# 001camellia/Speech-Imagery-EEG

Measured on AMD Instinct MI355X. Metric: epochs/sec (B=256, C=122, T=1000) IGN 3-class, higher is better.
Workload: dtype f32

## Files before the change

### speech-imagery-eeg_amd/csrc/ign_clconv.h

```cpp
#pragma once
#include "ign_common.h"

typedef float f32x16 __attribute__((ext_vector_type(16)));
#define MFMA32(a, b, c) __builtin_amdgcn_mfma_f32_32x32x2f32((a), (b), (c), 0, 0, 0)

__device__ __forceinline__ int acc_row16(int r, int h) { return (r & 3) + 8 * (r >> 2) + 4 * h; }

constexpr int TM = 128, TN = 128, KC = 16;
constexpr int NT_PITCH = KC + 4;
constexpr int TN_PITCH = 128 + 8;

struct RowMap {
    int rows_logical;
    int row0;
    int row_pitch;
    long long sample_pitch;
};
__device__ __forceinline__ long long row_off(const RowMap& rm, int m) {
    const int s = m / rm.rows_logical;
    const int r = m - s * rm.rows_logical;
    return (long long)s * rm.sample_pitch + (long long)(rm.row0 + r) * rm.row_pitch;
}

template <int V> struct VecT;
template <> struct VecT<1> { typedef float T; };
template <> struct VecT<2> { typedef float2 T; };
template <> struct VecT<4> { typedef float4 T; };

template <int V>
__device__ __forceinline__ void vload(float (&d)[V], const float* p) {
    if (V == 4) { const float4 t = *reinterpret_cast<const float4*>(p); d[0] = t.x; d[1] = t.y; d[2] = t.z; d[3] = t.w; }
    else if (V == 2) { const float2 t = *reinterpret_cast<const float2*>(p); d[0] = t.x; d[1] = t.y; }
    else d[0] = *p;
}
template <int V>
__device__ __forceinline__ void vstore(float* p, const float (&d)[V]) {
    if (V == 4) *reinterpret_cast<float4*>(p) = make_float4(d[0], d[1], d[2], d[3]);
    else if (V == 2) *reinterpret_cast<float2*>(p) = make_float2(d[0], d[1]);
    else *p = d[0];
}

enum { EPI_BIAS_STATS = 0, EPI_MASK_STATS = 1, EPI_GELU_BWD = 2 };

__device__ __forceinline__ float ign_gelu_grad(float u) {
    const float cdf = 0.5f * (1.f + erff(u * 0.70710678118654752f));
    const float pdf = 0.3989422804014327f * expf(-0.5f * u * u);
    return fmaf(u, pdf, cdf);
}

struct GemmNTArgs {
    const float* A; RowMap am; int K;
    const float* Bt; int ldb;
    float* C; int M, N;
    const float* bias;
    const float* pro_a; const float* pro_b; int pro_c;
    float* part;
    const float* ey; const float* ea; const float* eb; const float* emean; const float* einv;
    int mtiles, ntiles;
    const unsigned short* B3; int Kp;
    float* amax_out;
};

template <int EPI, bool FULL, bool SC = false>
__device__ __forceinline__ void nt_epilogue_body(const GemmNTArgs& a, const f32x16 (&acc)[2][2], float (&s1)[2], float (&s2)[2],
                                                 int m0, int n0, int m_lim, float osc = 1.f) {
    const int lane = threadIdx.x & 63, wave = threadIdx.x >> 6;
    const int l31 = lane & 31, h = lane >> 5;
    const int wm = wave & 1, wn = wave >> 1;
    float amax = 0.f;
#pragma unroll
    for (int j = 0; j < 2; ++j) {
        const int n = n0 + wn * 64 + j * 32 + l31;
        const bool n_ok = FULL || n < a.N;
        const int nc = n_ok ? n : a.N - 1;
        const float bv = (EPI == EPI_BIAS_STATS && a.bias) ? a.bias[nc] : 0.f;
        float ea = 0.f, eb = 0.f, em = 0.f, ei = 0.f;
        if (EPI == EPI_MASK_STATS) { ea = a.ea[nc]; eb = a.eb[nc]; em = a.emean[nc]; ei = a.einv[nc]; }
#pragma unroll
        for (int i = 0; i < 2; ++i) {
            const int mb = m0 + wm * 64 + i * 32;
            float yv[16];
            if (EPI == EPI_MASK_STATS || EPI == EPI_GELU_BWD) {
#pragma unroll
                for (int r = 0; r < 16; ++r) {
                    const int m = mb + acc_row16(r, h);
                    const int mc = FULL ? m : min(m, m_lim - 1);
                    yv[r] = a.ey[(long long)mc * a.N + nc];
                }
            }
#pragma unroll
            for (int r = 0; r < 16; ++r) {
                const int m = mb + acc_row16(r, h);
                const bool ok = FULL || (n_ok && m < m_lim);
                float v = SC ? acc[i][j][r] * osc : acc[i][j][r];
                if (EPI == EPI_BIAS_STATS) {
                    v += bv;
                    if (ok) { s1[j] += v; s2[j] = fmaf(v, v, s2[j]); }
                } else if (EPI == EPI_GELU_BWD) {
                    v *= ign_gelu_grad(yv[r]);
                } else {
                    v = (fmaf(ea, yv[r], eb) > 0.f) ? v : 0.f;
                    if (ok) { s1[j] += v; s2[j] = fmaf(v, (yv[r] - em) * ei, s2[j]); }
                }
                if (ok) a.C[(long long)m * a.N + n] = v;
                if (SC && ok) amax = fmaxf(amax, fabsf(v));
            }
        }
    }
    if (SC && a.amax_out) {
#pragma unroll
        for (int o = 32; o > 0; o >>= 1) amax = fmaxf(amax, __shfl_xor(amax, o, 64));
        if (lane == 0) ign_atomic_absmax(a.amax_out, amax);
    }
}

template <int EPI, bool SC = false>
__device__ __forceinline__ void nt_epilogue(const GemmNTArgs& a, const f32x16 (&acc)[2][2], float* red, int mt, int m0, int n0,
                                            int m_lim, float osc = 1.f) {
    const int tid = threadIdx.x, lane = tid & 63, wave = tid >> 6;
    const int l31 = lane & 31, h = lane >> 5;
    const int wm = wave & 1, wn = wave >> 1;
    float s1[2] = {0.f, 0.f}, s2[2] = {0.f, 0.f};
    if (m0 + TM <= m_lim && n0 + TN <= a.N) nt_epilogue_body<EPI, true, SC>(a, acc, s1, s2, m0, n0, m_lim, osc);
    else nt_epilogue_body<EPI, false, SC>(a, acc, s1, s2, m0, n0, m_lim, osc);
    if (a.part) {
#pragma unroll
        for (int j = 0; j < 2; ++j) {
            s1[j] += __shfl_xor(s1[j], 32, 64);
            s2[j] += __shfl_xor(s2[j], 32, 64);
            if (h == 0) {
                const int col = wn * 64 + j * 32 + l31;
                red[(wm * 2 + 0) * TN + col] = s1[j];
                red[(wm * 2 + 1) * TN + col] = s2[j];
            }
        }
        __syncthreads();
        if (tid < TN && n0 + tid < a.N) {
            a.part[((long long)mt * 2 + 0) * a.N + n0 + tid] = red[0 * TN + tid] + red[2 * TN + tid];
            a.part[((long long)mt * 2 + 1) * a.N + n0 + tid] = red[1 * TN + tid] + red[3 * TN + tid];
        }
    }
}


struct ConvX6Args {
    GemmNTArgs g;
    long long sample_pitch;
    int rows_in;
    int cin, cp, k;
    int trows;
    int tps;
    int nprod;
    const float* bound_a;
    const float* bound_b;
};

__device__ __forceinline__ float ign_pow2_scale(const float* bound) {
    if (!bound) return 1.f;
    const float b = *bound;
    if (!(b > 0.f) || !(b < INFINITY)) return 1.f;
    int e;
    (void)frexpf(b, &e);
    e = 14 - e;
    e = e < -60 ? -60 : (e > 60 ? 60 : e);
    return ldexpf(1.f, e);
}

inline int ign_vec_width(int c) { return (c % 4 == 0) ? 4 : (c % 2 == 0) ? 2 : 1; }

int ign_clconv_launch_x6t(const ConvX6Args& a, int epi, int V, bool pro, hipStream_t s);
int ign_clconv_launch_wgrad_reduce(const float* part, float* dw_oik, int nsplit, int Co, int Ci, int k, hipStream_t s);
```

### speech-imagery-eeg_amd/csrc/ign_clconv_x6.hip

```cpp
#include "ign_clconv.h"

typedef __bf16 bf16x8 __attribute__((ext_vector_type(8)));
constexpr int X6_PITCH = KC + 8;
constexpr int X6_PLANE = TM * X6_PITCH;
constexpr int X6_BLOCK = 3 * TN * KC;

typedef float f32x2 __attribute__((ext_vector_type(2)));
typedef __bf16 bf16x2 __attribute__((ext_vector_type(2)));
__device__ __forceinline__ void split3_pair(f32x2 v, bf16x2& x0, bf16x2& x1, bf16x2& x2) {
    x0 = __builtin_convertvector(v, bf16x2);
    f32x2 r = v - __builtin_convertvector(x0, f32x2);
    x1 = __builtin_convertvector(r, bf16x2);
    r -= __builtin_convertvector(x1, f32x2);
    x2 = __builtin_convertvector(r, bf16x2);
}
template <int V>
__device__ __forceinline__ void split3_store(const float (&t)[V], __bf16* d, int plane);
template <>
__device__ __forceinline__ void split3_store<1>(const float (&t)[1], __bf16* d, int plane);
__device__ __forceinline__ void split3(float v, __bf16& x0, __bf16& x1, __bf16& x2) {
    x0 = (__bf16)v;
    float r = v - (float)x0;
    x1 = (__bf16)r;
    r -= (float)x1;
    x2 = (__bf16)r;
}
template <>
__device__ __forceinline__ void split3_store<1>(const float (&t)[1], __bf16* d, int plane) {
    __bf16 x0, x1, x2;
    split3(t[0], x0, x1, x2);
    d[0] = x0; d[plane] = x1; d[2 * plane] = x2;
}
template <>
__device__ __forceinline__ void split3_store<2>(const float (&t)[2], __bf16* d, int plane) {
    bf16x2 x0, x1, x2;
    split3_pair(f32x2{t[0], t[1]}, x0, x1, x2);
    *reinterpret_cast<bf16x2*>(d) = x0;
    *reinterpret_cast<bf16x2*>(d + plane) = x1;
    *reinterpret_cast<bf16x2*>(d + 2 * plane) = x2;
}
template <>
__device__ __forceinline__ void split3_store<4>(const float (&t)[4], __bf16* d, int plane) {
    typedef __bf16 bf16x4 __attribute__((ext_vector_type(4)));
    bf16x2 a0, a1, a2, b0, b1, b2;
    split3_pair(f32x2{t[0], t[1]}, a0, a1, a2);
    split3_pair(f32x2{t[2], t[3]}, b0, b1, b2);
    *reinterpret_cast<bf16x4*>(d) = __builtin_shufflevector(a0, b0, 0, 1, 2, 3);
    *reinterpret_cast<bf16x4*>(d + plane) = __builtin_shufflevector(a1, b1, 0, 1, 2, 3);
    *reinterpret_cast<bf16x4*>(d + 2 * plane) = __builtin_shufflevector(a2, b2, 0, 1, 2, 3);
}

typedef _Float16 f16x2 __attribute__((ext_vector_type(2)));
typedef _Float16 f16x4 __attribute__((ext_vector_type(4)));
typedef _Float16 f16x8 __attribute__((ext_vector_type(8)));
__device__ __forceinline__ void split2h_pair(f32x2 v, f16x2& x0, f16x2& x1) {
    x0 = __builtin_convertvector(v, f16x2);
    x1 = __builtin_convertvector(v - __builtin_convertvector(x0, f32x2), f16x2);
}
template <int V>
__device__ __forceinline__ void split2h_store(const float (&t)[V], __bf16* d, int plane) {
    _Float16* dh = reinterpret_cast<_Float16*>(d);
    if constexpr (V == 1) {
        const _Float16 x0 = (_Float16)t[0];
        dh[0] = x0; dh[plane] = (_Float16)(t[0] - (float)x0);
    } else if constexpr (V == 2) {
        f16x2 x0, x1;
        split2h_pair(f32x2{t[0], t[1]}, x0, x1);
        *reinterpret_cast<f16x2*>(dh) = x0;
        *reinterpret_cast<f16x2*>(dh + plane) = x1;
    } else {
        f16x2 a0, a1, b0, b1;
        split2h_pair(f32x2{t[0], t[1]}, a0, a1);
        split2h_pair(f32x2{t[2], t[3]}, b0, b1);
        *reinterpret_cast<f16x4*>(dh) = __builtin_shufflevector(a0, b0, 0, 1, 2, 3);
        *reinterpret_cast<f16x4*>(dh + plane) = __builtin_shufflevector(a1, b1, 0, 1, 2, 3);
    }
}

template <int V, int NP>
__device__ __forceinline__ void split_store(const float (&t)[V], __bf16* d, int plane) {
    if constexpr (NP == 3) {
        split3_store<V>(t, d, plane);
    } else if constexpr (NP == 2) {
        split2h_store<V>(t, d, plane);
    } else if constexpr (V == 1) {
        d[0] = (__bf16)t[0];
    } else if constexpr (V == 2) {
        *reinterpret_cast<bf16x2*>(d) = __builtin_convertvector(f32x2{t[0], t[1]}, bf16x2);
    } else {
        typedef __bf16 bf16x4 __attribute__((ext_vector_type(4)));
        const bf16x2 a = __builtin_convertvector(f32x2{t[0], t[1]}, bf16x2), b = __builtin_convertvector(f32x2{t[2], t[3]}, bf16x2);
        *reinterpret_cast<bf16x4*>(d) = __builtin_shufflevector(a, b, 0, 1, 2, 3);
    }
}

template <int NP>
__device__ __forceinline__ f32x16 mfma16(const bf16x8& a, const bf16x8& b, const f32x16& c) {
    if constexpr (NP == 2)
        return __builtin_amdgcn_mfma_f32_32x32x16_f16(__builtin_bit_cast(f16x8, a), __builtin_bit_cast(f16x8, b), c, 0, 0, 0);
    else
        return __builtin_amdgcn_mfma_f32_32x32x16_bf16(a, b, c, 0, 0, 0);
}

#ifndef IGN_H3_WAVES
#define IGN_H3_WAVES 3
#endif
constexpr int X6T_SPAN = TM + 15;
constexpr int X6T_APLANE = X6T_SPAN * X6_PITCH;

template <int NP> struct X6tLds {
    static constexpr int NPL = (NP == 2) ? 2 : 3;
    static constexpr int ABUF = NPL * X6T_APLANE, BBUF = NPL * X6_PLANE;
    static constexpr size_t BYTES = (size_t)2 * (ABUF + BBUF) * sizeof(unsigned short);
};
template <int NP, int EPI> struct X6tWaves { static constexpr int N = (NP == 2 && EPI == EPI_BIAS_STATS) ? IGN_H3_WAVES : 2; };
template <int V, bool PRO, int EPI, int NP>
__global__ void __launch_bounds__(256, (X6tWaves<NP, EPI>::N)) clconv_x6t_kernel(const ConvX6Args ca) {
    const GemmNTArgs& a = ca.g;
    constexpr int VPR = KC / V;
    constexpr int APASS = (X6T_SPAN * VPR + 255) / 256;
    constexpr int X6T_ABUF = X6tLds<NP>::ABUF, X6T_BBUF = X6tLds<NP>::BBUF;
    extern __shared__ __attribute__((aligned(16))) unsigned short smem16[];
    __bf16* Abuf = reinterpret_cast<__bf16*>(smem16);
    __bf16* Bbuf = Abuf + 2 * X6T_ABUF;

    const int nwg = a.mtiles * a.ntiles;
    int lid = blockIdx.x;
    {
        const int per = nwg / 8;
        if (lid < per * 8) lid = (lid & 7) * per + (lid >> 3);
    }
    const int mt = lid / a.ntiles, nt = lid - mt * a.ntiles;
    const int bi = mt / ca.tps, tt = mt - bi * ca.tps;
    const int t0 = tt * TM, n0 = nt * TN;
    const int tid = threadIdx.x, lane = tid & 63, wave = tid >> 6;
    const int l31 = lane & 31, h = lane >> 5;
    const int wm = wave & 1, wn = wave >> 1;
    const int span = TM + ca.k - 1;
    const int nvec = span * VPR;

    const float* abase = a.A + (long long)bi * ca.sample_pitch;
    const int brw = tid >> 1, bh = tid & 1;
    const unsigned short* bsrc = a.B3 + (size_t)nt * (size_t)(ca.cp / KC) * ca.k * X6_BLOCK + (size_t)brw * KC + 8 * bh;
    constexpr size_t bplane = (size_t)TN * KC;

    f32x16 acc[2][2];
#pragma unroll
    for (int i = 0; i < 2; ++i)
#pragma unroll
        for (int j = 0; j < 2; ++j)
#pragma unroll
            for (int r = 0; r < 16; ++r) acc[i][j][r] = 0.f;

    float ra[APASS][V];
    float pa[V], pb[V];
    bool a_ok = false;
    uint4 rb00, rb01 = {}, rb02 = {}, rb10, rb11 = {}, rb12 = {};
    const int ncc = ca.cp / KC;
    const int nstep = ncc * ca.k;

    const float sa = (NP == 2) ? ign_pow2_scale(ca.bound_a) : 1.f;
    const float osc = (NP == 2) ? 1.f / (sa * ign_pow2_scale(ca.bound_b)) : 1.f;
    auto aload = [&](int cc) {
        const int ch = cc * KC + (tid % VPR) * V;
        a_ok = ch < ca.cin;
        if (PRO && a_ok) {
            vload<V>(pa, a.pro_a + ch); vload<V>(pb, a.pro_b + ch);
            if constexpr (NP == 2) {
#pragma unroll
                for (int v = 0; v < V; ++v) { pa[v] *= sa; pb[v] *= sa; }
            }
        }
#pragma unroll
        for (int p = 0; p < APASS; ++p) {
            const int idx = tid + p * 256;
            const int row = idx / VPR;
            if (a_ok && idx < nvec) vload<V>(ra[p], abase + (long long)min(t0 + row, ca.rows_in - 1) * ca.cin + ch);
            else {
#pragma unroll
                for (int v = 0; v < V; ++v) ra[p][v] = 0.f;
            }
        }
    };
    auto astore = [&](int buf) {
        __bf16* st = Abuf + buf * X6T_ABUF;
#pragma unroll
        for (int p = 0; p < APASS; ++p) {
            const int idx = tid + p * 256;
            if (idx < nvec) {
                const int row = idx / VPR, q = idx - row * VPR;
                float tv[V];
#pragma unroll
                for (int v = 0; v < V; ++v) {
                    tv[v] = ra[p][v];
                    if (PRO && a_ok) tv[v] = fmaxf(fmaf(pa[v], tv[v], pb[v]), 0.f);
                    else if (NP == 2) tv[v] *= sa;
                }
                split_store<V, NP>(tv, st + row * X6_PITCH + q * V, X6T_APLANE);
            }
        }
    };
    auto boff = [&](int st) {
        st = min(st, nstep - 1);
        return (size_t)st * X6_BLOCK;
    };
    auto bstore = [&](int buf, const uint4& r0, const uint4& r1, const uint4& r2) {
        __bf16* st = Bbuf + buf * X6T_BBUF + brw * X6_PITCH + 8 * bh;
        *reinterpret_cast<uint4*>(st) = r0;
        if constexpr (NP >= 2) *reinterpret_cast<uint4*>(st + X6_PLANE) = r1;
        if constexpr (NP == 3) *reinterpret_cast<uint4*>(st + 2 * X6_PLANE) = r2;
    };
#define IGN_BLOAD(r0, r1, r2, st)                                                                       \
    do {                                                                                                \
        const size_t off_ = boff(st);                                                                   \
        r0 = *reinterpret_cast<const uint4*>(bsrc + off_);                                              \
        if constexpr (NP >= 2) r1 = *reinterpret_cast<const uint4*>(bsrc + bplane + off_);              \
        if constexpr (NP == 3) r2 = *reinterpret_cast<const uint4*>(bsrc + 2 * bplane + off_);          \
    } while (0)

    aload(0);
    IGN_BLOAD(rb00, rb01, rb02, 0);
    IGN_BLOAD(rb10, rb11, rb12, 1);
    astore(0);
    bstore(0, rb00, rb01, rb02);
    __syncthreads();

    int cc = 0, j = 0;
    auto body = [&](int step, bool odd) {
        if (odd) IGN_BLOAD(rb10, rb11, rb12, step + 2);
        else IGN_BLOAD(rb00, rb01, rb02, step + 2);
        const bool next_span = cc + 1 < ncc;
        if (j == 0 && next_span) aload(cc + 1);
        const __bf16* As = Abuf + (cc & 1) * X6T_ABUF + (wm * 64 + l31 + j) * X6_PITCH + 8 * h;
        const __bf16* Bs = Bbuf + (step & 1) * X6T_BBUF + (wn * 64 + l31) * X6_PITCH + 8 * h;
        bf16x8 af[2][NP], bf[2][NP];
#pragma unroll
        for (int i = 0; i < 2; ++i)
#pragma unroll
            for (int pl = 0; pl < NP; ++pl) {
                af[i][pl] = *reinterpret_cast<const bf16x8*>(As + pl * X6T_APLANE + i * 32 * X6_PITCH);
                bf[i][pl] = *reinterpret_cast<const bf16x8*>(Bs + pl * X6_PLANE + i * 32 * X6_PITCH);
            }
        __builtin_amdgcn_sched_barrier(0);
#define IGN_X6(pa_, pb_)                                                                                   \
        acc[0][0] = mfma16<NP>(af[0][pa_], bf[0][pb_], acc[0][0]);                                         \
        acc[0][1] = mfma16<NP>(af[0][pa_], bf[1][pb_], acc[0][1]);                                         \
        acc[1][0] = mfma16<NP>(af[1][pa_], bf[0][pb_], acc[1][0]);                                         \
        acc[1][1] = mfma16<NP>(af[1][pa_], bf[1][pb_], acc[1][1]);
        if constexpr (NP == 3) { IGN_X6(2, 0) IGN_X6(0, 2) IGN_X6(1, 1) IGN_X6(1, 0) IGN_X6(0, 1) }
        if constexpr (NP == 2) { IGN_X6(1, 0) IGN_X6(0, 1) }
        IGN_X6(0, 0)
#undef IGN_X6
        __builtin_amdgcn_sched_barrier(0);
        if (odd) bstore((step + 1) & 1, rb00, rb01, rb02);
        else bstore((step + 1) & 1, rb10, rb11, rb12);
        if (j + 1 == ca.k) {
            if (next_span) astore((cc + 1) & 1);
            j = 0; ++cc;
        } else {
            ++j;
        }
        __syncthreads();
    };
    for (int step = 0; step < nstep; step += 2) {
        body(step, false);
        if (step + 1 < nstep) body(step + 1, true);
    }
#undef IGN_BLOAD
    const int m0 = bi * ca.trows + t0;
    nt_epilogue<EPI, NP == 2>(a, acc, reinterpret_cast<float*>(smem16), mt, m0, n0, bi * ca.trows + min(ca.trows, t0 + TM), osc);
}

#ifndef IGN_H3W_WAVES
#define IGN_H3W_WAVES 2
#endif
template <int NP> struct X6wLds {
    static constexpr int NPL = NP == 3 ? 3 : (NP == 2 ? 2 : 1);
    static constexpr int ABUF = NPL * TM * X6_PITCH;
    static constexpr int BBUF = 2 * NPL * X6_PLANE;
    static constexpr size_t BYTES = (size_t)2 * (ABUF + BBUF) * sizeof(unsigned short);
    static constexpr int WAVES = NP == 2 ? IGN_H3W_WAVES : 2;
};

template <int NP, int EPI = EPI_BIAS_STATS>
__global__ void __launch_bounds__(512, X6wLds<NP>::WAVES) clconv_x6w_kernel(const ConvX6Args ca) {
    const GemmNTArgs& a = ca.g;
    extern __shared__ __attribute__((aligned(16))) unsigned short smem16[];
    constexpr int X6W_ABUF = X6wLds<NP>::ABUF, X6W_BBUF = X6wLds<NP>::BBUF, NPL = X6wLds<NP>::NPL;
    __bf16* Abuf = reinterpret_cast<__bf16*>(smem16);
    __bf16* Bbuf = Abuf + 2 * X6W_ABUF;
    constexpr int APLANE = TM * X6_PITCH;

    const int ntw = a.N / 256;
    const int nwg = a.mtiles * ntw;
    int lid = blockIdx.x;
    {
        const int per = nwg / 8;
        if (lid < per * 8) lid = (lid & 7) * per + (lid >> 3);
    }
    const int mt = lid / ntw, nw = lid - mt * ntw;
    const int m0 = mt * TM, n0 = nw * 256;
    const int tid = threadIdx.x, lane = tid & 63, wave = tid >> 6;
    const int l31 = lane & 31, h = lane >> 5;
    const int wm = wave & 1, wn = wave >> 1;
    const int ncc = ca.cp / KC;

    f32x16 acc[2][2];
#pragma unroll
    for (int i = 0; i < 2; ++i)
#pragma unroll
        for (int j = 0; j < 2; ++j)
#pragma unroll
            for (int r = 0; r < 16; ++r) acc[i][j][r] = 0.f;

    const int arow = tid >> 2, ach = (tid & 3) * 4;
    const float* ap = a.A + (long long)min(m0 + arow, a.M - 1) * ca.cin + ach;
    float ra0[4], ra1[4];
    const int bt = tid >> 8, brw = (tid & 255) >> 1, bh = tid & 1;
    const unsigned short* bsrc = a.B3 + (size_t)(2 * nw + bt) * (size_t)ncc * X6_BLOCK + (size_t)brw * KC + 8 * bh;
    constexpr size_t bplane = (size_t)TN * KC;
    uint4 rb00, rb01 = {}, rb02 = {}, rb10, rb11 = {}, rb12 = {};

    const float sa = (NP == 2) ? ign_pow2_scale(ca.bound_a) : 1.f;
    const float osc = (NP == 2) ? 1.f / (sa * ign_pow2_scale(ca.bound_b)) : 1.f;
#define IGN_ALOADW(ra_, cc_)                                                                 \
    do {                                                                                     \
        const int c_ = min((cc_), ncc - 1);                                                  \
        if (c_ * KC + ach < ca.cin) vload<4>(ra_, ap + c_ * KC);           \
        else ra_[0] = ra_[1] = ra_[2] = ra_[3] = 0.f;                                        \
    } while (0)
    auto astore = [&](int buf, const float (&r)[4]) {
        if constexpr (NP == 2) {
            const float rs[4] = {r[0] * sa, r[1] * sa, r[2] * sa, r[3] * sa};
            split_store<4, NP>(rs, Abuf + buf * X6W_ABUF + arow * X6_PITCH + ach, APLANE);
        } else {
            split_store<4, NP>(r, Abuf + buf * X6W_ABUF + arow * X6_PITCH + ach, APLANE);
        }
    };
    auto bstore = [&](int buf, const uint4& r0, const uint4& r1, const uint4& r2) {
        __bf16* st = Bbuf + buf * X6W_BBUF + bt * NPL * X6_PLANE + brw * X6_PITCH + 8 * bh;
        *reinterpret_cast<uint4*>(st) = r0;
        if constexpr (NP >= 2) *reinterpret_cast<uint4*>(st + X6_PLANE) = r1;
        if constexpr (NP == 3) *reinterpret_cast<uint4*>(st + 2 * X6_PLANE) = r2;
    };
#define IGN_BLOADW(r0, r1, r2, st)                                                                      \
    do {                                                                                                \
        const size_t off_ = (size_t)min((st), ncc - 1) * X6_BLOCK;                                      \
        r0 = *reinterpret_cast<const uint4*>(bsrc + off_);                                              \
        if constexpr (NP >= 2) r1 = *reinterpret_cast<const uint4*>(bsrc + bplane + off_);              \
        if constexpr (NP == 3) r2 = *reinterpret_cast<const uint4*>(bsrc + 2 * bplane + off_);          \
    } while (0)

    IGN_ALOADW(ra0, 0);
    IGN_BLOADW(rb00, rb01, rb02, 0);
    IGN_ALOADW(ra1, 1);
    IGN_BLOADW(rb10, rb11, rb12, 1);
    astore(0, ra0);
    bstore(0, rb00, rb01, rb02);
    __syncthreads();

    const bool late = wave >= 4;
    auto mm = [&](int step) {
        const __bf16* As = Abuf + (step & 1) * X6W_ABUF + (wm * 64 + l31) * X6_PITCH + 8 * h;
        const __bf16* Bs = Bbuf + (step & 1) * X6W_BBUF + (wn >> 1) * NPL * X6_PLANE + ((wn & 1) * 64 + l31) * X6_PITCH + 8 * h;
        bf16x8 af[2][NP], bf[2][NP];
#pragma unroll
        for (int i = 0; i < 2; ++i)
#pragma unroll
            for (int pl = 0; pl < NP; ++pl) {
                af[i][pl] = *reinterpret_cast<const bf16x8*>(As + pl * APLANE + i * 32 * X6_PITCH);
                bf[i][pl] = *reinterpret_cast<const bf16x8*>(Bs + pl * X6_PLANE + i * 32 * X6_PITCH);
            }
        __builtin_amdgcn_sched_barrier(0);
#define IGN_X6(pa_, pb_)                                                                                   \
        acc[0][0] = mfma16<NP>(af[0][pa_], bf[0][pb_], acc[0][0]);                                         \
        acc[0][1] = mfma16<NP>(af[0][pa_], bf[1][pb_], acc[0][1]);                                         \
        acc[1][0] = mfma16<NP>(af[1][pa_], bf[0][pb_], acc[1][0]);                                         \
        acc[1][1] = mfma16<NP>(af[1][pa_], bf[1][pb_], acc[1][1]);
        if constexpr (NP == 3) { IGN_X6(2, 0) IGN_X6(0, 2) IGN_X6(1, 1) }
        if constexpr (NP >= 2) { IGN_X6(1, 0) IGN_X6(0, 1) }
        IGN_X6(0, 0)
#undef IGN_X6
        __builtin_amdgcn_sched_barrier(0);
    };
    auto body = [&](int step, bool odd) {
        if (odd) { IGN_BLOADW(rb10, rb11, rb12, step + 2); IGN_ALOADW(ra1, step + 2); }
        else { IGN_BLOADW(rb00, rb01, rb02, step + 2); IGN_ALOADW(ra0, step + 2); }
        const bool next = step + 1 < ncc;
        auto st = [&]() {
            if (odd) { bstore((step + 1) & 1, rb00, rb01, rb02); if (next) astore((step + 1) & 1, ra0); }
            else { bstore((step + 1) & 1, rb10, rb11, rb12); if (next) astore((step + 1) & 1, ra1); }
            __builtin_amdgcn_sched_barrier(0);
        };
        if (late) { st(); mm(step); } else { mm(step); st(); }
        __syncthreads();
    };
    for (int step = 0; step < ncc; step += 2) {
        body(step, false);
        if (step + 1 < ncc) body(step + 1, true);
    }
#undef IGN_BLOADW
#undef IGN_ALOADW
    float s1[2] = {0.f, 0.f}, s2[2] = {0.f, 0.f};
    const int m_lim = a.M;
    if (m0 + TM <= m_lim) nt_epilogue_body<EPI, true, NP == 2>(a, acc, s1, s2, m0, n0, m_lim, osc);
    else nt_epilogue_body<EPI, false, NP == 2>(a, acc, s1, s2, m0, n0, m_lim, osc);
}

__device__ __forceinline__ void pack_weights_x3t_body(const float* __restrict__ w, unsigned short* __restrict__ wt3,
                                                      unsigned short* __restrict__ wd3, int Co, int Ci, int k, int Cip, int Cop,
                                                      long long i, const float* __restrict__ bound = nullptr) {
    const long long nf = (long long)((Co + TN - 1) / TN) * (Cip / KC) * k * (TN * KC);
    const long long nd = wd3 ? (long long)((Ci + TN - 1) / TN) * (Cop / KC) * k * (TN * KC) : 0;
    const bool fwd = i < nf;
    if (!fwd && i >= nf + nd) return;
    const long long e = fwd ? i : i - nf;
    const int q = (int)(e % KC);
    long long t = e / KC;
    const int row = (int)(t % TN);
    t /= TN;
    const int j = (int)(t % k);
    t /= k;
    const int ncc = (fwd ? Cip : Cop) / KC;
    const int cc = (int)(t % ncc);
    const int nt = (int)(t / ncc);
    const int n = nt * TN + row, c = cc * KC + q;
    float v = 0.f;
    if (fwd) { if (n < Co && c < Ci) v = w[((long long)n * Ci + c) * k + j]; }
    else     { if (n < Ci && c < Co) v = w[((long long)c * Ci + n) * k + (k - 1 - j)]; }
    const long long blk = ((long long)(nt * ncc + cc) * k + j) * X6_BLOCK + (long long)row * KC + q;
    if (bound) {
        const float sv = v * ign_pow2_scale(bound);
        const _Float16 h0 = (_Float16)sv;
        _Float16* dh = reinterpret_cast<_Float16*>(fwd ? wt3 : wd3) + blk;
        dh[0] = h0; dh[TN * KC] = (_Float16)(sv - (float)h0);
        return;
    }
    __bf16 x0, x1, x2;
    split3(v, x0, x1, x2);
    __bf16* dst = reinterpret_cast<__bf16*>(fwd ? wt3 : wd3) + blk;
    dst[0] = x0; dst[TN * KC] = x1; dst[2 * TN * KC] = x2;
}

__global__ void __launch_bounds__(256) pack_weights_x3t_kernel(const float* __restrict__ w, unsigned short* __restrict__ wt3,
                                                               unsigned short* __restrict__ wd3, int Co, int Ci, int k, int Cip,
                                                               int Cop) {
    pack_weights_x3t_body(w, wt3, wd3, Co, Ci, k, Cip, Cop, (long long)blockIdx.x * 256 + threadIdx.x);
}

constexpr int PACK_LMAX = 8;
struct PackMultiTable {
    const float* w[PACK_LMAX];
    unsigned short* wt3[PACK_LMAX];
    unsigned short* wd3[PACK_LMAX];
    long long* counter[PACK_LMAX];
    const float* bound[PACK_LMAX];
    int Co[PACK_LMAX], Ci[PACK_LMAX], k[PACK_LMAX];
};
__global__ void __launch_bounds__(256) pack_weights_x3t_multi_kernel(const PackMultiTable t) {
    const int l = blockIdx.y;
    if (blockIdx.x == 0 && threadIdx.x == 0 && t.counter[l]) *t.counter[l] += 1;
    pack_weights_x3t_body(t.w[l], t.wt3[l], t.wd3[l], t.Co[l], t.Ci[l], t.k[l], (t.Ci[l] + 15) / 16 * 16, (t.Co[l] + 15) / 16 * 16,
                          (long long)blockIdx.x * 256 + threadIdx.x, t.bound[l]);
}

typedef short s16x4 __attribute__((ext_vector_type(4)));
typedef short s16x8 __attribute__((ext_vector_type(8)));
constexpr int WG_PITCH = 64 + 32;

struct WgradX6Args {
    const float* dy; long long dy_sample_pitch; int dy_row0;
    const float* x; long long x_sample_pitch;
    const float* pro_a; const float* pro_b;
    float* part;
    int B, Tin, Tout, Ci, Co, k;
    int cps;
    int nunits, nsplit, citiles;
    const float* bound_dy; const float* bound_x;
};

__device__ __forceinline__ bf16x8 lds_tr8(const __bf16* p0, const __bf16* p1) {
    typedef __attribute__((address_space(3))) s16x4* lds_p;
    const s16x4 lo = __builtin_amdgcn_ds_read_tr16_b64_v4i16((lds_p)(p0));
    const s16x4 hi = __builtin_amdgcn_ds_read_tr16_b64_v4i16((lds_p)(p1));
    const s16x8 v = __builtin_shufflevector(lo, hi, 0, 1, 2, 3, 4, 5, 6, 7);
    return __builtin_bit_cast(bf16x8, v);
}

template <int KT, int NR, int VX, bool PRO, int NP>
__global__ void __launch_bounds__(256, ((NP == 2 && KT <= 5) ? IGN_H3_WAVES : 2)) clconv_wgrad_x6_kernel(const WgradX6Args a) {
    constexpr int RU = 16 * NR;
    constexpr int SPAN = RU + KT - 1;
    constexpr int PPLANE = RU * WG_PITCH, QPLANE = SPAN * WG_PITCH;
    constexpr int NPL = (NP == 2) ? 2 : 3;
    constexpr int STAGE = NPL * (PPLANE + QPLANE);
    constexpr int XVPR = 64 / VX;
    constexpr int XPASS = (SPAN * XVPR + 255) / 256;
    constexpr int DPASS = NR;
    extern __shared__ __attribute__((aligned(16))) unsigned short smem16[];
    __bf16* smem = reinterpret_cast<__bf16*>(smem16);

    const int tile = blockIdx.x;
    const int cot = tile / a.citiles, cit = tile - cot * a.citiles;
    const int co0 = cot * 64, ci0 = cit * 64;
    const int split = blockIdx.y;
    const int per = (a.nunits + a.nsplit - 1) / a.nsplit;
    const int u_begin = split * per, u_end = min(a.nunits, u_begin + per);

    const int tid = threadIdx.x, lane = tid & 63, wave = tid >> 6;
    const int l31 = lane & 31, h = lane >> 5;
    const int wco = wave & 1, wci = wave >> 1;

    const int dr = tid >> 4, dc = (tid & 15) * 4;
    const bool d_ok = co0 + dc < a.Co;
    const int xq = (tid % XVPR) * VX;
    const bool x_ok = ci0 + xq < a.Ci;
    float pa[VX], pb[VX];
    if (PRO && x_ok) { vload<VX>(pa, a.pro_a + ci0 + xq); vload<VX>(pb, a.pro_b + ci0 + xq); }
    const float sdy = (NP == 2) ? ign_pow2_scale(a.bound_dy) : 1.f;
    const float sx = (NP == 2) ? ign_pow2_scale(a.bound_x) : 1.f;
    const float osc = (NP == 2) ? 1.f / (sdy * sx) : 1.f;
    if (NP == 2 && PRO && x_ok) {
#pragma unroll
        for (int v = 0; v < VX; ++v) { pa[v] *= sx; pb[v] *= sx; }
    }

    f32x16 acc[KT];
#pragma unroll
    for (int j = 0; j < KT; ++j)
#pragma unroll
        for (int r = 0; r < 16; ++r) acc[j][r] = 0.f;

    float rd[DPASS][4], rx[XPASS][VX];
    auto gload = [&](int u) {
        const int b = u / a.cps, t0 = (u - b * a.cps) * RU;
        const float* dyb = a.dy + (long long)b * a.dy_sample_pitch + (long long)a.dy_row0 * a.Co + co0 + dc;
        const float* xb = a.x + (long long)b * a.x_sample_pitch + ci0 + xq;
#pragma unroll
        for (int p = 0; p < DPASS; ++p) {
            const int t = t0 + dr + 16 * p;
            if (d_ok && t < a.Tout) vload<4>(rd[p], dyb + (long long)t * a.Co);
            else { rd[p][0] = rd[p][1] = rd[p][2] = rd[p][3] = 0.f; }
        }
#pragma unroll
        for (int p = 0; p < XPASS; ++p) {
            const int row = (tid + p * 256) / XVPR;
            if (x_ok && row < SPAN) vload<VX>(rx[p], xb + (long long)min(t0 + row, a.Tin - 1) * a.Ci);
            else {
#pragma unroll
                for (int v = 0; v < VX; ++v) rx[p][v] = 0.f;
            }
        }
    };
    auto lstore = [&](int buf) {
        __bf16* P = smem + buf * STAGE;
        __bf16* Q = P + NPL * PPLANE;
#pragma unroll
        for (int p = 0; p < DPASS; ++p) {
            if constexpr (NP == 2) {
#pragma unroll
                for (int v = 0; v < 4; ++v) rd[p][v] *= sdy;
            }
            split_store<4, NP>(rd[p], P + (dr + 16 * p) * WG_PITCH + dc, PPLANE);
        }
#pragma unroll
        for (int p = 0; p < XPASS; ++p) {
            const int row = (tid + p * 256) / XVPR;
            if (row < SPAN) {
                float tv[VX];
#pragma unroll
                for (int v = 0; v < VX; ++v) {
// ... 490 lines not shown
```

Before: 2.864.

## Stream conv weight tiles via direct global-to-LDS DMA in a three-stage ring

Replaces the register-staged double-buffered weight (B) loads in the x6t conv kernel with global_load_lds direct-to-LDS copies into a three-slot ring. Synchronisation uses explicit vmcnt waits plus s_barrier instead of __syncthreads. This is meant to remove the register round trip and LDS store instructions from the main loop. The epilogue also switches to tile-relative addressing with a scalarised wave index, and the NP==2 occupancy setting now applies to every epilogue type, not just bias-stats. Risks are hand-written vmcnt counts that must match the number of outstanding loads, and an unpadded B layout in LDS that may cause bank conflicts.

```diff
diff --git a/speech-imagery-eeg_amd/csrc/ign_clconv.h b/speech-imagery-eeg_amd/csrc/ign_clconv.h
--- a/speech-imagery-eeg_amd/csrc/ign_clconv.h
+++ b/speech-imagery-eeg_amd/csrc/ign_clconv.h
@@ -64,7 +64,7 @@
 template <int EPI, bool FULL, bool SC = false>
 __device__ __forceinline__ void nt_epilogue_body(const GemmNTArgs& a, const f32x16 (&acc)[2][2], float (&s1)[2], float (&s2)[2],
                                                  int m0, int n0, int m_lim, float osc = 1.f) {
-    const int lane = threadIdx.x & 63, wave = threadIdx.x >> 6;
+    const int lane = threadIdx.x & 63, wave = __builtin_amdgcn_readfirstlane(threadIdx.x >> 6);
     const int l31 = lane & 31, h = lane >> 5;
     const int wm = wave & 1, wn = wave >> 1;
     float amax = 0.f;
@@ -79,18 +79,21 @@
 #pragma unroll
         for (int i = 0; i < 2; ++i) {
             const int mb = m0 + wm * 64 + i * 32;
+            const long long tile0 = (long long)mb * a.N + n0;
+            const unsigned loff = (unsigned)(4 * h) * (unsigned)a.N + (unsigned)(nc - n0);
             float yv[16];
             if (EPI == EPI_MASK_STATS || EPI == EPI_GELU_BWD) {
 #pragma unroll
                 for (int r = 0; r < 16; ++r) {
-                    const int m = mb + acc_row16(r, h);
-                    const int mc = FULL ? m : min(m, m_lim - 1);
-                    yv[r] = a.ey[(long long)mc * a.N + nc];
+                    const int r0 = acc_row16(r, 0);
+                    if (FULL) yv[r] = (a.ey + (tile0 + (long long)r0 * a.N))[loff];
+                    else yv[r] = (a.ey + tile0)[min(r0 + 4 * h, m_lim - 1 - mb) * a.N + (nc - n0)];
                 }
             }
 #pragma unroll
             for (int r = 0; r < 16; ++r) {
-                const int m = mb + acc_row16(r, h);
+                const int r0 = acc_row16(r, 0);
+                const int m = mb + r0 + 4 * h;
                 const bool ok = FULL || (n_ok && m < m_lim);
                 float v = SC ? acc[i][j][r] * osc : acc[i][j][r];
                 if (EPI == EPI_BIAS_STATS) {
@@ -102,9 +105,10 @@
                     v = (fmaf(ea, yv[r], eb) > 0.f) ? v : 0.f;
                     if (ok) { s1[j] += v; s2[j] = fmaf(v, (yv[r] - em) * ei, s2[j]); }
                 }
-                if (ok) a.C[(long long)m * a.N + n] = v;
+                if (ok) (a.C + (tile0 + (long long)r0 * a.N))[loff] = v;
                 if (SC && ok) amax = fmaxf(amax, fabsf(v));
             }
+            if (EPI == EPI_MASK_STATS) __builtin_amdgcn_sched_barrier(0);
         }
     }
     if (SC && a.amax_out) {
diff --git a/speech-imagery-eeg_amd/csrc/ign_clconv_x6.hip b/speech-imagery-eeg_amd/csrc/ign_clconv_x6.hip
--- a/speech-imagery-eeg_amd/csrc/ign_clconv_x6.hip
+++ b/speech-imagery-eeg_amd/csrc/ign_clconv_x6.hip
@@ -111,15 +111,17 @@
 template <int NP> struct X6tLds {
     static constexpr int NPL = (NP == 2) ? 2 : 3;
     static constexpr int ABUF = NPL * X6T_APLANE, BBUF = NPL * X6_PLANE;
+    static constexpr int BSTAGE = NP * TN * KC;
+    static_assert(3 * BSTAGE <= 2 * BBUF, "the three-stage weight ring must fit the two padded stages it replaces");
     static constexpr size_t BYTES = (size_t)2 * (ABUF + BBUF) * sizeof(unsigned short);
 };
-template <int NP, int EPI> struct X6tWaves { static constexpr int N = (NP == 2 && EPI == EPI_BIAS_STATS) ? IGN_H3_WAVES : 2; };
+template <int NP, int EPI> struct X6tWaves { static constexpr int N = (NP == 2) ? IGN_H3_WAVES : 2; };
 template <int V, bool PRO, int EPI, int NP>
 __global__ void __launch_bounds__(256, (X6tWaves<NP, EPI>::N)) clconv_x6t_kernel(const ConvX6Args ca) {
     const GemmNTArgs& a = ca.g;
     constexpr int VPR = KC / V;
     constexpr int APASS = (X6T_SPAN * VPR + 255) / 256;
-    constexpr int X6T_ABUF = X6tLds<NP>::ABUF, X6T_BBUF = X6tLds<NP>::BBUF;
+    constexpr int X6T_ABUF = X6tLds<NP>::ABUF;
     extern __shared__ __attribute__((aligned(16))) unsigned short smem16[];
     __bf16* Abuf = reinterpret_cast<__bf16*>(smem16);
     __bf16* Bbuf = Abuf + 2 * X6T_ABUF;
@@ -140,8 +142,9 @@
     const int nvec = span * VPR;
 
     const float* abase = a.A + (long long)bi * ca.sample_pitch;
-    const int brw = tid >> 1, bh = tid & 1;
-    const unsigned short* bsrc = a.B3 + (size_t)nt * (size_t)(ca.cp / KC) * ca.k * X6_BLOCK + (size_t)brw * KC + 8 * bh;
+    constexpr int BSTAGE = X6tLds<NP>::BSTAGE;
+    const int wv = __builtin_amdgcn_readfirstlane(wave);
+    const unsigned short* bsrc = a.B3 + (size_t)nt * (size_t)(ca.cp / KC) * ca.k * X6_BLOCK + (size_t)(wv * 32 + l31) * KC + 8 * h;
     constexpr size_t bplane = (size_t)TN * KC;
 
     f32x16 acc[2][2];
@@ -155,7 +158,6 @@
     float ra[APASS][V];
     float pa[V], pb[V];
     bool a_ok = false;
-    uint4 rb00, rb01 = {}, rb02 = {}, rb10, rb11 = {}, rb12 = {};
     const int ncc = ca.cp / KC;
     const int nstep = ncc * ca.k;
 
@@ -200,46 +202,48 @@
             }
         }
     };
-    auto boff = [&](int st) {
-        st = min(st, nstep - 1);
-        return (size_t)st * X6_BLOCK;
-    };
-    auto bstore = [&](int buf, const uint4& r0, const uint4& r1, const uint4& r2) {
-        __bf16* st = Bbuf + buf * X6T_BBUF + brw * X6_PITCH + 8 * bh;
-        *reinterpret_cast<uint4*>(st) = r0;
-        if constexpr (NP >= 2) *reinterpret_cast<uint4*>(st + X6_PLANE) = r1;
-        if constexpr (NP == 3) *reinterpret_cast<uint4*>(st + 2 * X6_PLANE) = r2;
-    };
-#define IGN_BLOAD(r0, r1, r2, st)                                                                       \
-    do {                                                                                                \
-        const size_t off_ = boff(st);                                                                   \
-        r0 = *reinterpret_cast<const uint4*>(bsrc + off_);                                              \
-        if constexpr (NP >= 2) r1 = *reinterpret_cast<const uint4*>(bsrc + bplane + off_);              \
-        if constexpr (NP == 3) r2 = *reinterpret_cast<const uint4*>(bsrc + 2 * bplane + off_);          \
-    } while (0)
+    auto bdma = [&](int st, int slot) {
+        typedef __attribute__((address_space(1))) const void* gptr_t;
+        typedef __attribute__((address_space(3))) void* lptr_t;
+        const unsigned short* g = bsrc + (size_t)st * X6_BLOCK;
+        __bf16* d = Bbuf + slot * BSTAGE + wv * (32 * KC);
+#pragma unroll
+        for (int pl = 0; pl < NP; ++pl)
+            __builtin_amdgcn_global_load_lds((gptr_t)(g + pl * bplane), (lptr_t)(d + pl * (TN * KC)), 16, 0, 0);
+    };
+    auto step_sync = [&](bool more) {
+        if (more) {
+            if constexpr (NP == 3) asm volatile("s_waitcnt vmcnt(3) lgkmcnt(0)" ::: "memory");
+            else if constexpr (NP == 2) asm volatile("s_waitcnt vmcnt(2) lgkmcnt(0)" ::: "memory");
+            else asm volatile("s_waitcnt vmcnt(1) lgkmcnt(0)" ::: "memory");
+        } else {
+            asm volatile("s_waitcnt vmcnt(0) lgkmcnt(0)" ::: "memory");
+        }
+        __builtin_amdgcn_s_barrier();
+        asm volatile("" ::: "memory");
+    };
 
     aload(0);
-    IGN_BLOAD(rb00, rb01, rb02, 0);
-    IGN_BLOAD(rb10, rb11, rb12, 1);
+    bdma(0, 0);
+    if (nstep > 1) bdma(1, 1);
     astore(0);
-    bstore(0, rb00, rb01, rb02);
-    __syncthreads();
-
-    int cc = 0, j = 0;
-    auto body = [&](int step, bool odd) {
-        if (odd) IGN_BLOAD(rb10, rb11, rb12, step + 2);
-        else IGN_BLOAD(rb00, rb01, rb02, step + 2);
+    step_sync(nstep > 1);
+
+    int cc = 0, j = 0, rs = 0;
+    for (int step = 0; step < nstep; ++step) {
         const bool next_span = cc + 1 < ncc;
         if (j == 0 && next_span) aload(cc + 1);
+        const bool more = step + 2 < nstep;
+        if (more) bdma(step + 2, rs == 0 ? 2 : rs - 1);
         const __bf16* As = Abuf + (cc & 1) * X6T_ABUF + (wm * 64 + l31 + j) * X6_PITCH + 8 * h;
-        const __bf16* Bs = Bbuf + (step & 1) * X6T_BBUF + (wn * 64 + l31) * X6_PITCH + 8 * h;
+        const __bf16* Bs = Bbuf + rs * BSTAGE + wn * (64 * KC) + lane * 8;
         bf16x8 af[2][NP], bf[2][NP];
 #pragma unroll
         for (int i = 0; i < 2; ++i)
 #pragma unroll
             for (int pl = 0; pl < NP; ++pl) {
                 af[i][pl] = *reinterpret_cast<const bf16x8*>(As + pl * X6T_APLANE + i * 32 * X6_PITCH);
-                bf[i][pl] = *reinterpret_cast<const bf16x8*>(Bs + pl * X6_PLANE + i * 32 * X6_PITCH);
+                bf[i][pl] = *reinterpret_cast<const bf16x8*>(Bs + pl * (TN * KC) + i * (32 * KC));
             }
         __builtin_amdgcn_sched_barrier(0);
 #define IGN_X6(pa_, pb_)                                                                                   \
@@ -252,21 +256,15 @@
         IGN_X6(0, 0)
 #undef IGN_X6
         __builtin_amdgcn_sched_barrier(0);
-        if (odd) bstore((step + 1) & 1, rb00, rb01, rb02);
-        else bstore((step + 1) & 1, rb10, rb11, rb12);
         if (j + 1 == ca.k) {
             if (next_span) astore((cc + 1) & 1);
             j = 0; ++cc;
         } else {
             ++j;
         }
-        __syncthreads();
-    };
-    for (int step = 0; step < nstep; step += 2) {
-        body(step, false);
-        if (step + 1 < nstep) body(step + 1, true);
-    }
-#undef IGN_BLOAD
+        rs = rs == 2 ? 0 : rs + 1;
+        step_sync(more);
+    }
     const int m0 = bi * ca.trows + t0;
     nt_epilogue<EPI, NP == 2>(a, acc, reinterpret_cast<float*>(smem16), mt, m0, n0, bi * ca.trows + min(ca.trows, t0 + TM), osc);
 }
```

After: 2.878 (median of 6 runs). No clear change (+0.5%).
